# dongxianzhe/hydrainfer

Hardware: AMD Instinct MI355X
Metric: decode output tokens/s, LLaVA-1.5-7B image+text requests (576 image + 128 text prompt, 256 generated), batch 32 per GPU (higher is better)
Workload: dtype bf16; 1 GPU; LLaVA-1.5-7B-shaped random weights, batch 32 decode, paged KV block_size=16, 613 steps in 3 passes of consecutive contexts (the generation's 705..959, the last pass ctx 781..883), the state rewound between passes outside the clock (BASELINE configs[1]: LLaVA-1.5-7B bf16, collocated prefill+decode on 1 MI355X); global_batch=32, hip_graph=False, step_executor=plan, parallelism=replicas x1 (independent requests, no data-path collective)

## Files before the change

### hydrainfer_amd/csrc/gemm_xreg.hip

```cpp
#include <algorithm>
#include <cstdio>
#include <cstdlib>
#include <cstring>
#include <type_traits>
#include "attn_common.h"

namespace {

using namespace hx;

struct XregParams {
  const void* x;
  const void* w;
  float* partial;
  int64_t ldx;
  int32_t M, N, K;
  int32_t stagger;
  int32_t x_packed;
  const float* nm_partial;
  void* nm_residual;
  const void* nm_weight;
  uint32_t* sync;
  int32_t nm_splits;
  float nm_eps;
  void* act;
  int32_t interleaved;
  int32_t pk_P;
};

struct XregHot {
  const void *p0, *p1, *p2, *p3, *p4;
  int32_t a, b, c, ldx;
};
template <int NORM>
inline bool xreg_hot(const XregParams& p, unsigned nb, XregHot* h) {
  if ((p.N >> 4) > 0xffff || nb > 0xffff || (p.K >> 5) > 0xffff || p.M > 255 || p.nm_splits > 255 || p.stagger > 255 ||
      p.pk_P > 0xffff || p.pk_P < 0 || p.ldx > 0x7fffffff || p.ldx < 0)
    return false;
  h->p0 = p.w;
  if (NORM) { h->p1 = p.nm_partial; h->p2 = p.nm_residual; h->p3 = p.nm_weight; h->p4 = p.sync; }
  else { h->p1 = p.x; h->p2 = p.partial; h->p3 = p.act; h->p4 = nullptr; }
  h->a = (int32_t)((uint32_t)(p.N >> 4) | (nb << 16));
  h->b = (int32_t)((uint32_t)(p.K >> 5) | ((uint32_t)p.M << 16) | ((uint32_t)(p.x_packed ? 1 : 0) << 24) | ((uint32_t)(p.interleaved ? 1 : 0) << 25));
  h->c = (int32_t)((uint32_t)p.stagger | ((uint32_t)p.nm_splits << 8) | ((uint32_t)p.pk_P << 16));
  h->ldx = NORM ? __builtin_bit_cast(int32_t, p.nm_eps) : (int32_t)p.ldx;
  return true;
}

#define HX_XREG_HOT_SIG                                                                                             \
  const void* __restrict__ h_p0, const void* __restrict__ h_p1, const void* __restrict__ h_p2,                        \
      const void* __restrict__ h_p3, const void* __restrict__ h_p4, const int32_t h_a, const int32_t h_b,            \
      const int32_t h_c, const int32_t h_ldx
#define HX_XREG_UNPACK_HOT(NORM_)                                                                                   \
  XregParams p = p_in;                                                                                              \
  p.w = h_p0;                                                                                                       \
  if (NORM_) {                                                                                                      \
    p.nm_partial = reinterpret_cast<const float*>(h_p1); p.nm_residual = const_cast<void*>(h_p2); p.nm_weight = h_p3; \
    p.sync = reinterpret_cast<uint32_t*>(const_cast<void*>(h_p4));                                                  \
  } else {                                                                                                          \
    p.x = h_p1; p.partial = reinterpret_cast<float*>(const_cast<void*>(h_p2)); p.act = const_cast<void*>(h_p3);     \
  }                                                                                                                 \
  p.N = (h_a & 0xffff) << 4; p.K = (h_b & 0xffff) << 5; p.M = (h_b >> 16) & 0xff; p.x_packed = (h_b >> 24) & 1;     \
  p.interleaved = (h_b >> 25) & 1; p.stagger = h_c & 0xff; p.nm_splits = (h_c >> 8) & 0xff;                         \
  p.pk_P = (int32_t)((uint32_t)h_c >> 16);                                                                          \
  if (NORM_) p.nm_eps = __builtin_bit_cast(float, h_ldx);                                                           \
  else p.ldx = h_ldx;                                                                                               \
  const int h_nb = (int)((uint32_t)h_a >> 16);

__device__ __forceinline__ float silu_f32(float x) { return x / (1.0f + __expf(-x)); }

__device__ __attribute__((aligned(128))) u16 g_zero_line[64] = {0};

static_assert(HX_XREG_SYNC_WORDS >= 320 + 32, "sync area: word 0 arrivals, word 1 error, word 32*(1+xcc) the flag line of that XCD");
constexpr int kXAux = 16;
constexpr int kStateWord = 320;
constexpr uint64_t kRescueTicks = 3000;
constexpr int kMaxG = 16;

typedef __amdgpu_buffer_rsrc_t rsrc_t;
typedef unsigned int bu32x4 __attribute__((__vector_size__(16)));
__device__ __forceinline__ rsrc_t make_rsrc(const void* p) {
  return __builtin_amdgcn_make_buffer_rsrc(const_cast<void*>(p), 0, 0x7fffffff, 0x00020000);
}

template <typename T, int MAXV, int MB, int KB = 6>
__device__ __forceinline__ bool norm_row_256(const float* __restrict__ partial, int n_splits, int64_t slab_stride,
                                             u16* __restrict__ residual, const u16* __restrict__ weight, float eps,
                                             int hidden, int row, void* x_frag, uint32_t* state, float* red,
                                             int mb_layout = MB) {
  const int tid = threadIdx.x;
  const int nvec = hidden / 8;
  uint32_t claimed = 1;
  if (tid == 0) claimed = __hip_atomic_exchange(state + row, 1u, __ATOMIC_RELAXED, __HIP_MEMORY_SCOPE_AGENT);
  u16x8* res_v = reinterpret_cast<u16x8*>(residual + (int64_t)row * hidden);
  const u16x8* w_v = reinterpret_cast<const u16x8*>(weight);
  float x[2 * MAXV][8];
  float ss[2] = {0.f, 0.f};
  u16x8 rr[2 * MAXV], ww[2 * MAXV], hh[2 * MAXV];
#pragma unroll
  for (int v = 0; v < 2; ++v)
#pragma unroll
    for (int j = 0; j < MAXV; ++j) {
      const int i = min(tid + 256 * v + 512 * j, nvec - 1);
      rr[v * MAXV + j] = res_v[i];
      ww[v * MAXV + j] = w_v[i];
    }
#pragma unroll
  for (int v = 0; v < 2; ++v) {
#pragma unroll
    for (int j = 0; j < MAXV; ++j) {
      const int i = tid + 256 * v + 512 * j;
      if (i < nvec) {
        const float* pp = partial + (int64_t)row * hidden + i * 8;
        constexpr int kB = KB;
        f32x4 a = {0.f, 0.f, 0.f, 0.f}, b = {0.f, 0.f, 0.f, 0.f};
        for (int s0 = 0; s0 < n_splits; s0 += kB) {
          f32x4 pa[kB], pb[kB];
#pragma unroll
          for (int k = 0; k < kB; ++k) {
            const int sp = min(s0 + k, n_splits - 1);
            pa[k] = *reinterpret_cast<const f32x4*>(pp + sp * slab_stride);
            pb[k] = *reinterpret_cast<const f32x4*>(pp + sp * slab_stride + 4);
          }
#pragma unroll
          for (int k = 0; k < kB; ++k) {
            if (s0 + k == 0) { a = pa[0]; b = pb[0]; }
            else if (s0 + k < n_splits) { a += pa[k]; b += pb[k]; }
          }
        }
        const u16x8 r = rr[v * MAXV + j];
        u16x8 h;
#pragma unroll
        for (int e = 0; e < 8; ++e) {
          const float sum = round_to<T>(round_to<T>(e < 4 ? a[e] : b[e - 4]) + T::to_float(r[e]));
          x[v * MAXV + j][e] = sum;
          h[e] = T::from_float(sum);
          ss[v] += sum * sum;
        }
        hh[v * MAXV + j] = h;
      }
    }
  }
  const float t0 = wave_sum(ss[0]), t1 = wave_sum(ss[1]);
  if ((tid & 63) == 0) {
    red[tid >> 6] = t0;
    red[4 + (tid >> 6)] = t1;
  }
  if (tid == 0) red[8] = claimed == 0u ? 1.f : 0.f;
  __syncthreads();
  const bool own = red[8] != 0.f;
  float total = 0.f;
#pragma unroll
  for (int k = 0; k < 8; ++k) total += red[k];
  const float inv = rsqrtf(total / (float)hidden + eps);
  if (own) {
    const rsrc_t xrs = make_rsrc(x_frag);
#pragma unroll
    for (int v = 0; v < 2; ++v) {
#pragma unroll
      for (int j = 0; j < MAXV; ++j) {
        const int i = tid + 256 * v + 512 * j;
        if (i < nvec) {
          res_v[i] = hh[v * MAXV + j];
          const u16x8 w = ww[v * MAXV + j];
          u16x8 o;
#pragma unroll
          for (int e = 0; e < 8; ++e)
            o[e] = T::from_float(round_to<T>(x[v * MAXV + j][e] * inv) * T::to_float(w[e]));
          const uint32_t piece = (uint32_t)((i >> 2) * mb_layout + (row >> 4)) * 64 + (i & 3) * 16 + (row & 15);
          __builtin_amdgcn_raw_buffer_store_b128(__builtin_bit_cast(bu32x4, o), xrs, piece * 16, 0, 16);
        }
      }
    }
  }
  __syncthreads();
  return own;
}

template <typename T, int MB, int KW, int EPI = 0, int DBG = 0, int NORM = 0, int RM = 0>
__global__ __launch_bounds__(256) void gemm_xreg_kernel(HX_XREG_HOT_SIG, const XregParams p_in) {
  HX_XREG_UNPACK_HOT(NORM)
  extern __shared__ __attribute__((aligned(16))) char smem[];
  constexpr int NBUF = (KW + 7) / 8;
  constexpr int P = 4 * KW;
  const int lane = threadIdx.x & 63;
  const int w = __builtin_amdgcn_readfirstlane(threadIdx.x >> 6);
  const int g = lane >> 4, c = lane & 15;
  const int split = blockIdx.y, nb = h_nb, b = nb - 1 - (int)blockIdx.x;
  const int total_ks = p.K >> 5;
  const int n_rg = p.N >> 4;
  const int ks0 = split * P;
  const int nks = min(P, total_ks - ks0);
  const int kw = max(0, min(KW, nks - w * KW));
  const int G = EPI ? 2 * (((n_rg >> 1) - b + nb - 1) / nb) : (n_rg - b + nb - 1) / nb;
  auto rg_of = [&](int i) { return EPI ? 2 * (b + (i >> 1) * nb) + (i & 1) : b + i * nb; };
  const int j0 = (p.stagger & 1) ? (int)(((unsigned)b * 7u + (unsigned)w * 3u) % (unsigned)KW) : 0;
  const int flat_id = blockIdx.y * nb + blockIdx.x;
  auto stamp = [&](int k) {
    if (NORM && (p.stagger & 8) && threadIdx.x == 0 && (flat_id == 0 || flat_id == (int)(nb * (NORM ? 1u : gridDim.y)) - 1))
      reinterpret_cast<unsigned long long*>(p.sync + 384 + (flat_id ? 32 : 0))[k] = __builtin_amdgcn_s_memrealtime();
  };
  stamp(0);

  auto rot = [&](int t) { const int r = j0 + t; return r >= KW ? r - KW : r; };
  constexpr int64_t jstride = RM ? 32 : 512;
  const u16* wbase = RM ? reinterpret_cast<const u16*>(p.w) + (int64_t)c * p.K + 8 * g + (int64_t)ks0 * 32
                        : reinterpret_cast<const u16*>(p.w) + 8 * lane + ((int64_t)ks0 * n_rg) * 512;
  auto rg_off = [&](int rg) -> int64_t {
    if constexpr (!RM) return (int64_t)rg * nks * 512;
    else if (EPI || p.interleaved) return ((int64_t)(rg & 1) * (p.N >> 1) + (int64_t)(rg >> 1) * 16) * p.K;
    else return (int64_t)rg * 16 * p.K;
  };
  const int wave_k0 = min(w * KW, max(nks - 1, 0));
  auto frag_ptr = [&](int rg, int t) {
    const int r = rot(t);
    const int j = wave_k0 + (r < kw ? r : 0);
    return wbase + rg_off(rg) + j * jstride;
  };

  u16x8 buf[NBUF][8];
  auto load_buf = [&](int rg, int q) {
#pragma unroll
    for (int j = 0; j < 8; ++j)
      if (8 * q + j < KW) buf[q][j] = __builtin_nontemporal_load(reinterpret_cast<const u16x8*>(frag_ptr(rg, 8 * q + j)));
  };
  u16x8 xb[KW][MB];
  const u16* xp = reinterpret_cast<const u16*>(p.x) + 8 * g;
  const u16* zp = reinterpret_cast<const u16*>(g_zero_line) + 8 * g;
  auto load_x_block = [&](int q) {
#pragma unroll
    for (int j = 0; j < 8; ++j) {
      const int t = 8 * q + j;
      if (t < KW) {
        const int r = rot(t);
        const bool ok = r < kw;
        const int ks = min(ks0 + w * KW + r, total_ks - 1);
#pragma unroll
        for (int mb = 0; mb < MB; ++mb) {
          const int m = min(mb * 16 + c, p.M - 1);
          const u16* src = ok ? (p.x_packed ? reinterpret_cast<const u16*>(p.x) + ((int64_t)(ks * MB + mb) * 64 + lane) * 8
                                            : xp + (int64_t)m * p.ldx + (int64_t)ks * 32)
                              : zp;
          if (DBG & 1) xb[t][mb] = u16x8{1, 2, 3, 4, 5, 6, (u16)t, (u16)lane};
          else xb[t][mb] = *reinterpret_cast<const u16x8*>(src);
        }
      }
    }
  };
  if (NORM) {
    uint32_t* st = p.sync + kStateWord;
    float* red = reinterpret_cast<float*>(smem);
    int* cmd = reinterpret_cast<int*>(smem) + 16;
    auto produce = [&](int row) {
      const bool own = norm_row_256<T, (KW + 31) / 32, MB>(p.nm_partial, p.nm_splits, (int64_t)p.M * p.K,
                                                           reinterpret_cast<u16*>(p.nm_residual),
                                                           reinterpret_cast<const u16*>(p.nm_weight), p.nm_eps, p.K, row,
                                                           const_cast<void*>(p.x), st, red);
      if (own) {
        asm volatile("s_waitcnt vmcnt(0)" ::: "memory");
        __syncthreads();
        if (threadIdx.x == 0) {
          const uint32_t old = __hip_atomic_fetch_add(p.sync, 1u, __ATOMIC_RELAXED, __HIP_MEMORY_SCOPE_AGENT);
          if (old + 1 == (uint32_t)p.M) {
#pragma unroll
            for (int cpy = 0; cpy < 8; ++cpy)
              __hip_atomic_store(p.sync + 32 * (1 + cpy), 1u, __ATOMIC_RELAXED, __HIP_MEMORY_SCOPE_AGENT);
          }
        }
      }
      return own;
    };
    const int flat = flat_id;
    const int n_wg = nb;
    if (flat < p.M && !(p.stagger & 6))
      for (int row = flat; row < p.M; row += n_wg) produce(row);
    stamp(1);
#pragma unroll
    for (int q = 0; q < NBUF; ++q) load_buf(rg_of(0), q);
    __builtin_amdgcn_sched_barrier(0);
    for (;;) {
      if (threadIdx.x < 64) {
        const uint32_t* fl = p.sync + 32 * (1 + (__builtin_amdgcn_s_getreg(20 | (3 << 11)) & 7));
        const uint64_t t0 = __builtin_amdgcn_s_memrealtime();
        int c = -1;
        while (!__builtin_amdgcn_readfirstlane(__hip_atomic_load(fl, __ATOMIC_RELAXED, __HIP_MEMORY_SCOPE_AGENT))) {
          __builtin_amdgcn_s_sleep(8);
          const uint64_t waited = __builtin_amdgcn_s_memrealtime() - t0;
          if (waited > kRescueTicks && !(p.stagger & 4)) {
            const uint32_t sv = lane < p.M ? __hip_atomic_load(st + lane, __ATOMIC_RELAXED, __HIP_MEMORY_SCOPE_AGENT) : 1u;
            uint64_t free_rows = __ballot(sv == 0u);
            if (free_rows) {
              for (int skip = flat % __builtin_popcountll(free_rows); skip > 0; --skip) free_rows &= free_rows - 1;
              c = __builtin_ctzll(free_rows);
              break;
            }
          }
          if (waited > ((p.stagger & 4) ? 200000ull : 100000000ull)) {
            if (threadIdx.x == 0) __hip_atomic_fetch_or(p.sync + 1, 1u, __ATOMIC_RELAXED, __HIP_MEMORY_SCOPE_AGENT);
            c = -2;
            break;
          }
        }
        if (threadIdx.x == 0) *cmd = c;
      }
      __syncthreads();
      const int c = *cmd;
      __syncthreads();
      if (c < 0) break;
      produce(c);
    }
    stamp(2);
    asm volatile("" ::: "memory");
    {
      const rsrc_t xrs = make_rsrc(p.x), zrs = make_rsrc(g_zero_line);
#pragma unroll
      for (int t = 0; t < KW; ++t) {
        const int r = rot(t);
        const bool ok = r < kw;
        const int ks = min(ks0 + w * KW + r, total_ks - 1);
#pragma unroll
        for (int mb = 0; mb < MB; ++mb) {
          xb[t][mb] = __builtin_bit_cast(u16x8, __builtin_amdgcn_raw_buffer_load_b128(
              ok ? xrs : zrs, ok ? (uint32_t)((ks * MB + mb) * 64 + lane) * 16 : (uint32_t)(lane & 7) * 16, 0, kXAux));
        }
      }
    }
    __builtin_amdgcn_sched_barrier(0);
  } else {
#pragma unroll
    for (int q = 0; q < NBUF; ++q) {
      load_x_block(q);
      load_buf(rg_of(0), q);
      __builtin_amdgcn_sched_barrier(0);
    }
  }

  f32x4 acc[MB];
#pragma unroll
  for (int mb = 0; mb < MB; ++mb) acc[mb] = f32x4{0.f, 0.f, 0.f, 0.f};
  f32x4* slot = reinterpret_cast<f32x4*>(smem) + (w * MB) * 64 + lane;

  auto row_group = [&](int i, auto refill_tag) {
    constexpr bool REFILL = decltype(refill_tag)::value;
    const int rg_next = rg_of(i + 1);
#pragma unroll
    for (int q = 0; q < NBUF; ++q) {
#pragma unroll
      for (int j = 0; j < 8; ++j) {
        if (8 * q + j < KW) {
#pragma unroll
          for (int mb = 0; mb < MB; ++mb) acc[mb] = Mfma<T>::mma(buf[q][j], xb[8 * q + j][mb], acc[mb]);
        }
      }
      __builtin_amdgcn_sched_barrier(0);
      if (REFILL) load_buf(rg_next, q);
      __builtin_amdgcn_sched_barrier(0);
    }
#pragma unroll
    for (int mb = 0; mb < MB; ++mb) {
      slot[(i * 4 * MB + mb) * 64] = acc[mb];
      acc[mb] = f32x4{0.f, 0.f, 0.f, 0.f};
    }
  };
  for (int i = 0; i < G - 1; ++i) { row_group(i, std::true_type{}); if (i < 6) stamp(3 + i); }
  row_group(G - 1, std::false_type{});
  stamp(10);
  if ((DBG & 2) && acc[0][0] != 123.25f) return;
  __syncthreads();

  const f32x4* tiles = reinterpret_cast<const f32x4*>(smem) + lane;
  auto tile_sum = [&](int i, int mb) {
    f32x4 s = tiles[((i * 4 + 0) * MB + mb) * 64];
#pragma unroll
    for (int ww = 1; ww < 4; ++ww) s += tiles[((i * 4 + ww) * MB + mb) * 64];
    return s;
  };
  if (EPI == 0) {
    for (int pr = w; pr < G * MB; pr += 4) {
      const int i = pr / MB, mb = pr - i * MB;
      const f32x4 s = tile_sum(i, mb);
      const int m = mb * 16 + c;
      const int rg = rg_of(i);
      const int col = p.interleaved ? ((rg & 1) ? (p.N >> 1) : 0) + ((rg >> 1) << 4) : (rg << 4);
      if (m < p.M) *reinterpret_cast<f32x4*>(p.partial + ((int64_t)split * p.M + m) * p.N + col + 4 * g) = s;
    }
  } else {
    for (int pr = w; pr < (G >> 1) * MB; pr += 4) {
      const int ip = pr / MB, mb = pr - ip * MB;
      const f32x4 gt = tile_sum(2 * ip, mb), up = tile_sum(2 * ip + 1, mb);
      u16x4 r;
#pragma unroll
      for (int e = 0; e < 4; ++e)
        r[e] = T::from_float(round_to<T>(silu_f32(round_to<T>(gt[e]))) * round_to<T>(up[e]));
      const int k = 16 * (b + ip * nb) + 4 * g;
      u16* dst = reinterpret_cast<u16*>(p.act) + ((((int64_t)(k >> 5) * MB + mb) * 64 + ((k & 31) >> 3) * 16 + c) << 3) + (k & 7);
      *reinterpret_cast<u16x4*>(dst) = r;
    }
  }
  stamp(11);
}

template <typename T, int KW, int NORM, int RG = 2, int EPI = 0>
__global__ __launch_bounds__(256) void gemm_xreg_wide_kernel(HX_XREG_HOT_SIG, const XregParams p_in) {
  HX_XREG_UNPACK_HOT(NORM)
  extern __shared__ __attribute__((aligned(16))) char smem[];
  constexpr int MB = 4, NBUF = (KW + 7) / 8, P = 4 * KW;
  static_assert(!EPI || (RG == 2 && NORM == 1), "the two-pass form: (gate, up) pairs, norm-fused");
  const int lane = threadIdx.x & 63;
  const int w = __builtin_amdgcn_readfirstlane(threadIdx.x >> 6);
  const int g = lane >> 4, c = lane & 15;
  const int split = EPI ? 0 : (int)blockIdx.y, nb = h_nb, b = nb - 1 - (int)blockIdx.x;
  const int total_ks = p.K >> 5;
  const int n_rg = p.N >> 4, n_un = n_rg / RG;
  const int sp = split >> 1, off_in = (split & 1) * P;
  const int nks_p = min(p.pk_P, total_ks - sp * p.pk_P);
  const int ks0 = sp * p.pk_P + off_in;
  const int nks = max(0, min(P, nks_p - off_in));
  const int kw = max(0, min(KW, nks - w * KW));
  const int G = (n_un - b + nb - 1) / nb;
  const int mbl = (p.M + 15) >> 4;
  const int j0 = (p.stagger & 1) ? (int)(((unsigned)b * 7u + (unsigned)w * 3u) % (unsigned)KW) : 0;
  const int flat_id = blockIdx.y * nb + blockIdx.x;
  auto stamp = [&](int k) {
    if (NORM && (p.stagger & 8) && threadIdx.x == 0 && (flat_id == 0 || flat_id == (int)(nb * gridDim.y) - 1))
      reinterpret_cast<unsigned long long*>(p.sync + 384 + (flat_id ? 32 : 0))[k] = __builtin_amdgcn_s_memrealtime();
  };
  stamp(0);
  auto rot = [&](int t) { const int r = j0 + t; return r >= KW ? r - KW : r; };
  const u16* wbase = reinterpret_cast<const u16*>(p.w) + 8 * lane + ((int64_t)sp * p.pk_P * n_rg) * 512;
  const int wave_k0 = off_in + min(w * KW, max(nks - 1, 0));
  struct PassK { int ks0, kw, wk0; };
  const PassK pa{ks0, kw, wave_k0};
  const int nks_b = max(0, min(P, nks_p - P));
  const PassK pb{ks0 + P, max(0, min(KW, nks_b - w * KW)), P + min(w * KW, max(nks_b - 1, 0))};
  auto frag_ptr = [&](int rg, int t, const PassK& ps) {
    const int r = rot(t);
    return wbase + ((int64_t)rg * nks_p + ps.wk0 + (r < ps.kw ? r : 0)) * 512;
  };
  u16x8 buf[RG][NBUF][8];
  auto load_buf = [&](int unit, int q, const PassK& ps) {
#pragma unroll
    for (int h = 0; h < RG; ++h)
#pragma unroll
      for (int j = 0; j < 8; ++j)
        if (8 * q + j < KW)
          buf[h][q][j] = __builtin_nontemporal_load(reinterpret_cast<const u16x8*>(frag_ptr(RG * unit + h, 8 * q + j, ps)));
  };
  auto unit_of = [&](int i) { return b + i * nb; };
  u16x8 xb[KW][MB];
  const u16* xp = reinterpret_cast<const u16*>(p.x) + 8 * g;
  const u16* zp = reinterpret_cast<const u16*>(g_zero_line) + 8 * g;
  auto load_x_block = [&](int q) {
#pragma unroll
    for (int j = 0; j < 8; ++j) {
      const int t = 8 * q + j;
      if (t < KW) {
        const int r = rot(t);
        const bool ok = r < kw;
        const int ks = min(ks0 + w * KW + r, total_ks - 1);
#pragma unroll
        for (int mb = 0; mb < MB; ++mb) {
          const int m = min(mb * 16 + c, p.M - 1);
          const u16* src = ok ? (p.x_packed ? reinterpret_cast<const u16*>(p.x) + ((int64_t)(ks * mbl + min(mb, mbl - 1)) * 64 + lane) * 8
                                            : xp + (int64_t)m * p.ldx + (int64_t)ks * 32)
                              : zp;
          xb[t][mb] = *reinterpret_cast<const u16x8*>(src);
        }
      }
    }
  };
  if (NORM) {
    uint32_t* st = p.sync + kStateWord;
    float* red = reinterpret_cast<float*>(smem);
    int* cmd = reinterpret_cast<int*>(smem) + 16;
    auto produce = [&](int row) {
      const bool own = norm_row_256<T, (2 * KW + 31) / 32, MB, 8>(p.nm_partial, p.nm_splits, (int64_t)p.M * p.K,
                                                               reinterpret_cast<u16*>(p.nm_residual),
                                                               reinterpret_cast<const u16*>(p.nm_weight), p.nm_eps, p.K, row,
                                                               const_cast<void*>(p.x), st, red, mbl);
      if (own) {
        asm volatile("s_waitcnt vmcnt(0)" ::: "memory");
        __syncthreads();
        if (threadIdx.x == 0) {
          const uint32_t old = __hip_atomic_fetch_add(p.sync, 1u, __ATOMIC_RELAXED, __HIP_MEMORY_SCOPE_AGENT);
          if (old + 1 == (uint32_t)p.M) {
#pragma unroll
            for (int cpy = 0; cpy < 8; ++cpy)
              __hip_atomic_store(p.sync + 32 * (1 + cpy), 1u, __ATOMIC_RELAXED, __HIP_MEMORY_SCOPE_AGENT);
          }
        }
      }
      return own;
    };
    const int n_wg = nb * (int)gridDim.y;
    if (flat_id < p.M && !(p.stagger & 6))
      for (int row = flat_id; row < p.M; row += n_wg) produce(row);
#pragma unroll
    for (int q = 0; q < NBUF; ++q) load_buf(unit_of(0), q, pa);
    __builtin_amdgcn_sched_barrier(0);
    stamp(1);
    for (;;) {
      if (threadIdx.x < 64) {
        const uint32_t* fl = p.sync + 32 * (1 + (__builtin_amdgcn_s_getreg(20 | (3 << 11)) & 7));
        const uint64_t t0 = __builtin_amdgcn_s_memrealtime();
        int cc = -1;
        while (!__builtin_amdgcn_readfirstlane(__hip_atomic_load(fl, __ATOMIC_RELAXED, __HIP_MEMORY_SCOPE_AGENT))) {
          __builtin_amdgcn_s_sleep(8);
          const uint64_t waited = __builtin_amdgcn_s_memrealtime() - t0;
          if (waited > kRescueTicks && !(p.stagger & 4)) {
            const uint32_t sv = lane < p.M ? __hip_atomic_load(st + lane, __ATOMIC_RELAXED, __HIP_MEMORY_SCOPE_AGENT) : 1u;
            uint64_t free_rows = __ballot(sv == 0u);
            if (free_rows) {
              for (int skip = flat_id % __builtin_popcountll(free_rows); skip > 0; --skip) free_rows &= free_rows - 1;
              cc = __builtin_ctzll(free_rows);
              break;
            }
          }
          if (waited > ((p.stagger & 4) ? 200000ull : 100000000ull)) {
            if (threadIdx.x == 0) __hip_atomic_fetch_or(p.sync + 1, 1u, __ATOMIC_RELAXED, __HIP_MEMORY_SCOPE_AGENT);
            cc = -2;
            break;
          }
        }
        if (threadIdx.x == 0) *cmd = cc;
      }
      __syncthreads();
      const int cc = *cmd;
      __syncthreads();
      if (cc < 0) break;
      produce(cc);
    }
    stamp(2);
    asm volatile("" ::: "memory");
  }
  auto load_x_norm = [&](const PassK& ps) {
    const rsrc_t xrs = make_rsrc(p.x), zrs = make_rsrc(g_zero_line);
#pragma unroll
    for (int t = 0; t < KW; ++t) {
      const int r = rot(t);
      const bool ok = r < ps.kw;
      const int ks = min(ps.ks0 + w * KW + r, total_ks - 1);
#pragma unroll
      for (int mb = 0; mb < MB; ++mb)
        xb[t][mb] = __builtin_bit_cast(u16x8, __builtin_amdgcn_raw_buffer_load_b128(
            ok ? xrs : zrs, ok ? (uint32_t)((ks * mbl + min(mb, mbl - 1)) * 64 + lane) * 16 : (uint32_t)(lane & 7) * 16, 0, kXAux));
    }
  };
  if (NORM) {
    load_x_norm(pa);
    __builtin_amdgcn_sched_barrier(0);
  } else {
#pragma unroll
    for (int q = 0; q < NBUF; ++q) {
      load_x_block(q);
      load_buf(unit_of(0), q, pa);
      __builtin_amdgcn_sched_barrier(0);
    }
  }

  f32x4 acc[RG][MB];
#pragma unroll
  for (int h = 0; h < RG; ++h)
#pragma unroll
    for (int mb = 0; mb < MB; ++mb) acc[h][mb] = f32x4{0.f, 0.f, 0.f, 0.f};
  f32x4* tiles = reinterpret_cast<f32x4*>(smem) + lane;
  auto mfma_unit = [&](auto refill_tag, int u_next, const PassK& ps_next) {
    constexpr bool REFILL = decltype(refill_tag)::value;
#pragma unroll
    for (int q = 0; q < NBUF; ++q) {
#pragma unroll
      for (int j = 0; j < 8; ++j) {
        if (8 * q + j < KW) {
#pragma unroll
          for (int h = 0; h < RG; ++h)
#pragma unroll
            for (int mb = 0; mb < MB; ++mb) acc[h][mb] = Mfma<T>::mma(buf[h][q][j], xb[8 * q + j][mb], acc[h][mb]);
        }
      }
      __builtin_amdgcn_sched_barrier(0);
      if (REFILL) load_buf(u_next, q, ps_next);
      __builtin_amdgcn_sched_barrier(0);
    }
  };
  auto reduce_unit = [&](int set, f32x4 (&sum)[RG]) {
#pragma unroll
    for (int h = 0; h < RG; ++h)
#pragma unroll
      for (int mb = 0; mb < MB; ++mb) {
        tiles[(((set * RG + h) * 4 + w) * MB + mb) * 64] = acc[h][mb];
        acc[h][mb] = f32x4{0.f, 0.f, 0.f, 0.f};
      }
    __syncthreads();
#pragma unroll
    for (int k = 0; k < RG; ++k) {
      const int tt = w + 4 * k, h = tt >> 2, mb = tt & 3;
      sum[k] = tiles[(((set * RG + h) * 4 + 0) * MB + mb) * 64];
#pragma unroll
      for (int ww = 1; ww < 4; ++ww) sum[k] += tiles[(((set * RG + h) * 4 + ww) * MB + mb) * 64];
    }
  };
  if constexpr (!EPI) {
    auto unit = [&](int i, auto refill_tag) {
      mfma_unit(refill_tag, unit_of(i + 1), pa);
      f32x4 sum[RG];
      reduce_unit(i & 1, sum);
#pragma unroll
      for (int k = 0; k < RG; ++k) {
        const int tt = w + 4 * k, h = tt >> 2, mb = tt & 3;
        const int rg = RG * unit_of(i) + h;
        const int col = p.interleaved ? ((rg & 1) ? (p.N >> 1) : 0) + ((rg >> 1) << 4) : (rg << 4);
        const int m = mb * 16 + c;
        if (m < p.M) *reinterpret_cast<f32x4*>(p.partial + ((int64_t)split * p.M + m) * p.N + col + 4 * g) = sum[k];
      }
    };
    for (int i = 0; i < G - 1; ++i) { unit(i, std::true_type{}); if (i < 6) stamp(3 + i); }
    unit(G - 1, std::false_type{});
  } else {
    f32x4* part = reinterpret_cast<f32x4*>(smem + 2 * RG * 4 * MB * 1024) + lane;
    int n_red = 0;
    for (int i = 0; i < G; ++i) {
      const bool seam = i + 1 == G;
      mfma_unit(std::true_type{}, seam ? unit_of(0) : unit_of(i + 1), seam ? pb : pa);
      f32x4 sum[RG];
      reduce_unit(n_red++ & 1, sum);
#pragma unroll
      for (int k = 0; k < RG; ++k) part[((i * RG + k) * 4 + w) * 64] = sum[k];
      if (i < 3) stamp(3 + i);
    }
    load_x_norm(pb);
    __builtin_amdgcn_sched_barrier(0);
    auto finish = [&](int i, auto refill_tag) {
      mfma_unit(refill_tag, unit_of(i + 1), pb);
      f32x4 sum[RG];
      reduce_unit(n_red++ & 1, sum);
      f32x4 gt = part[((i * RG + 0) * 4 + w) * 64], up = part[((i * RG + 1) * 4 + w) * 64];
      gt += sum[0];
      up += sum[1];
      const int m = w * 16 + c;
      if (m < p.M) {
        u16x4 r;
#pragma unroll
        for (int e = 0; e < 4; ++e)
          r[e] = T::from_float(round_to<T>(silu_f32(round_to<T>(gt[e]))) * round_to<T>(up[e]));
        const int k = (unit_of(i) << 4) + 4 * g;
        u16* dst = reinterpret_cast<u16*>(p.act) + ((((int64_t)(k >> 5) * mbl + w) * 64 + ((k & 31) >> 3) * 16 + c) << 3) + (k & 7);
        *reinterpret_cast<u16x4*>(dst) = r;
      }
    };
    for (int i = 0; i < G - 1; ++i) { finish(i, std::true_type{}); if (i < 3) stamp(6 + i); }
    finish(G - 1, std::false_type{});
  }
  stamp(11);
}

__global__ __launch_bounds__(256) void pack_xreg_kernel(u16* __restrict__ packed, const u16* __restrict__ w,
                                                        int64_t n_pieces, int total_ks, int n_rg, int64_t ldw, int P,
                                                        int interleave) {
  const int64_t i = (int64_t)blockIdx.x * 256 + threadIdx.x;
  if (i >= n_pieces) return;
  const int lane = (int)(i & 63);
  const int64_t blk = i >> 6;
  const int64_t per_split = (int64_t)P * n_rg;
  const int split = (int)(blk / per_split);
  const int ks0 = split * P;
  const int nks = min(P, total_ks - ks0);
  const int64_t rem = blk - (int64_t)ks0 * n_rg;
  const int64_t rg = rem / nks;
  const int s = ks0 + (int)(rem % nks);
  const int64_t srg = interleave ? (rg >> 1) + ((rg & 1) ? (n_rg >> 1) : 0) : rg;
  const u16* src = w + (16 * srg + (lane & 15)) * ldw + 32 * s + 8 * (lane >> 4);
  *reinterpret_cast<u16x8*>(packed + i * 8) = *reinterpret_cast<const u16x8*>(src);
}

int g_stagger = 1;
int g_no_producers = 0;
int g_dbg = 0;
int g_row_major = 0;
int g_timeline = 0;
int g_force_wgs = 0;

constexpr int kKwSet[] = {4, 8, 16, 20, 22, 27, 29, 32, 40};

int round_kw(int kw) {
  for (int v : kKwSet) if (v >= kw) return v;
  return 0;
}

int n_cus() {
  static int n = [] {
    int dev = 0;
    hipDeviceProp_t prop;
    if (hipGetDevice(&dev) != hipSuccess || hipGetDeviceProperties(&prop, dev) != hipSuccess) return 256;
    return prop.multiProcessorCount > 0 ? prop.multiProcessorCount : 256;
  }();
  return n;
}

void xreg_plan(int64_t N, int64_t K, int* S, int* KW, bool fewest_splits = false) {
  const int total_ks = (int)(K >> 5);
  const int n_rg = (int)(N >> 4);
  const int s0 = (total_ks + 159) / 160;
  auto kw_of = [&](int s) { return round_kw(((total_ks + s - 1) / s + 3) / 4); };
  auto wgs_of = [&](int s) {
    int nb = n_cus() / s;
    if (nb < 1) nb = 1;
    if (nb > n_rg) nb = n_rg;
    const int G = (n_rg + nb - 1) / nb;
    return s * ((n_rg + G - 1) / G);
  };
  int s = s0;
  if (!fewest_splits) {
    auto waste_pct = [&](int sc) {
      const int kw = kw_of(sc);
      if (kw <= 0) return 1000;
      const int used = (total_ks + 4 * kw - 1) / (4 * kw);
      return used != sc ? 1000 : (int)(((int64_t)used * 4 * kw * 100) / total_ks) - 100;
    };
    const int w0 = waste_pct(s0), w1 = waste_pct(s0 + 1);
    if (w1 <= 4 && (w0 > 4 ||
                    (wgs_of(s0) * 5 < n_cus() * 4 && wgs_of(s0 + 1) > wgs_of(s0))))
      s = s0 + 1;
  }
  static const char* env = getenv("HX_XREG_S");
  if (env) {
    const char* q = env;
    while (*q) {
      long k = 0, sv = 0;
      if (sscanf(q, "%ld:%ld", &k, &sv) == 2 && k == K && sv >= s0 && sv <= 16) s = (int)sv;
      const char* semi = strchr(q, ';');
      if (!semi) break;
      q = semi + 1;
    }
  }
  *KW = kw_of(s);
  *S = *KW > 0 ? (total_ks + 4 * *KW - 1) / (4 * *KW) : 0;
}

template <typename T, int MB, int KW, int EPI, int NORM = 0>
int launch_kw(const XregParams& p, int S, hipStream_t stream) {
  const int n_units = EPI ? (p.N >> 5) : (p.N >> 4);
  const int per_unit = EPI ? 2 : 1;
  const int cap = g_force_wgs > 0 ? g_force_wgs : n_cus();
  int nb = cap / S;
  if (nb < 1) nb = 1;
  if (nb > n_units) nb = n_units;
  int G = (n_units + nb - 1) / nb;
  if (G * per_unit > kMaxG) {
    G = kMaxG / per_unit;
    nb = (n_units + G - 1) / G;
  }
  if (((n_units + nb - 1) / nb) * per_unit > kMaxG) return HX_ERR_SHAPE;
  const size_t lds = (size_t)G * per_unit * 4 * MB * 1024;
  if (lds > 48 * 1024) {
    hipError_t e = hipFuncSetAttribute((const void*)gemm_xreg_kernel<T, MB, KW, EPI, 0, NORM>,
                                       hipFuncAttributeMaxDynamicSharedMemorySize, (int)lds);
    if (e != hipSuccess) return hip_rc(e);
  }
  const dim3 grid((unsigned)nb, (unsigned)S);
  XregHot h;
  if (!xreg_hot<NORM>(p, (unsigned)nb, &h)) return HX_ERR_SHAPE;
  if (NORM && S != 1) return HX_ERR_SHAPE;
#define HX_XREG_LAUNCH(...) hx::launcher(gemm_xreg_kernel<__VA_ARGS__>, grid, 256, lds, stream)(h.p0, h.p1, h.p2, h.p3, h.p4, h.a, h.b, h.c, h.ldx, p)
  if constexpr (EPI == 0 && NORM == 0 && MB == 2 && (KW == 32 || KW == 29)) if (g_dbg) {
    if (g_dbg == 1) HX_XREG_LAUNCH(T, MB, KW, 0, 1);
    else if (g_dbg == 2) HX_XREG_LAUNCH(T, MB, KW, 0, 2);
    else HX_XREG_LAUNCH(T, MB, KW, 0, 3);
    return check_launch();
  }
#if HX_EXPERIMENTS
  if constexpr (MB == 2 && (KW == 32 || KW == 22 || KW == 29)) if (p.stagger & 16) {
    HX_XREG_LAUNCH(T, MB, KW, EPI, 0, NORM, 1);
    return check_launch();
  }
#endif
  HX_XREG_LAUNCH(T, MB, KW, EPI, 0, NORM);
#undef HX_XREG_LAUNCH
  return check_launch();
}

template <typename T, int MB, int EPI, int NORM = 0>
int launch_mb(const XregParams& p, int S, int KW, hipStream_t stream) {
  switch (KW) {
    case 4: return launch_kw<T, MB, 4, EPI, NORM>(p, S, stream);
    case 8: return launch_kw<T, MB, 8, EPI, NORM>(p, S, stream);
    case 16: return launch_kw<T, MB, 16, EPI, NORM>(p, S, stream);
    case 20: if constexpr (EPI == 0 && NORM == 0) return launch_kw<T, MB, 20, 0>(p, S, stream); else return HX_ERR_SHAPE;
    case 22: if constexpr (EPI == 0 && NORM == 0) return launch_kw<T, MB, 22, 0>(p, S, stream); else return HX_ERR_SHAPE;
    case 27: if constexpr (EPI == 0 && NORM == 0) return launch_kw<T, MB, 27, 0>(p, S, stream); else return HX_ERR_SHAPE;
    case 29: if constexpr (EPI == 0 && NORM == 0) return launch_kw<T, MB, 29, 0>(p, S, stream); else return HX_ERR_SHAPE;
    case 32: return launch_kw<T, MB, 32, EPI, NORM>(p, S, stream);
    case 40: return launch_kw<T, MB, 40, EPI, NORM>(p, S, stream);
    default: return HX_ERR_SHAPE;
  }
}

template <int EPI, int NORM = 0>
int launch_any(const XregParams& p, int S, int KW, int dtype, hipStream_t stream) {
  const int MB = (p.M + 15) / 16;
  if (dtype == HX_F16) return MB == 1 ? launch_mb<F16, 1, EPI, NORM>(p, S, KW, stream) : launch_mb<F16, 2, EPI, NORM>(p, S, KW, stream);
  return MB == 1 ? launch_mb<BF16, 1, EPI, NORM>(p, S, KW, stream) : launch_mb<BF16, 2, EPI, NORM>(p, S, KW, stream);
}

bool wide_plan(int64_t N, int64_t K, bool gate_up_packing, int* S, int* KW, int* pkP, int* S_packed) {
  if (N <= 0 || K <= 0 || N % 32 || K % 32) return false;
  int sp, kwp;
  xreg_plan(N, K, &sp, &kwp, gate_up_packing);
  if (kwp <= 0) return false;
  const int kw = (kwp + 1) / 2;
  if (kw != 2 && kw != 4 && kw != 8 && kw != 10 && kw != 11 && kw != 14 && kw != 16 && kw != 20) return false;
  const int total_ks = (int)(K >> 5);
  int n = 0;
  for (int q = 0; q < sp; ++q) {
    const int nks_p = std::min(4 * kwp, total_ks - q * 4 * kwp);
    n += nks_p > 4 * kw ? 2 : 1;
  }
  *KW = kw; *pkP = 4 * kwp; *S = n; *S_packed = sp;
  return true;
}

constexpr int wide_rg(int kw) { return kw == 20 ? 1 : 2; }

template <typename T, int KW, int NORM, int EPI = 0>
int launch_wide_kw(const XregParams& p, int S, hipStream_t stream) {
  constexpr int RG = wide_rg(KW);
  const int n_units = (int)(p.N >> 4) / RG;
  if (EPI) S = 1;
  int nb = n_cus() / S;
  if (nb < 1) nb = 1;
  if (nb > n_units) nb = n_units;
  size_t lds = 2 * RG * 4 * 4 * 1024;
  if (EPI) lds += (size_t)((n_units + nb - 1) / nb) * RG * 4 * 1024;
  if (lds > 150 * 1024) return HX_ERR_SHAPE;
  {
    hipError_t e = hipFuncSetAttribute((const void*)gemm_xreg_wide_kernel<T, KW, NORM, RG, EPI>,
// ... 359 lines not shown
```

Baseline: 6557 tokens/s.

## Replace block-wide flag wait with per-wave scalar polling and shared handover

The fused norm+GEMM kernel used to wait for the norm-ready flag with wave 0 polling and then two block barriers. Each wave now polls the flag itself with scalar glc loads. A small shared-memory handshake word escalates to a block barrier only when wave 0 decides to rescue a free row or give up. This is meant to remove the barrier round-trip from the common path so waves can start their GEMM as soon as the flag rises. In exchange it brings more complex cross-wave coordination with possible race risk, and more scalar memory traffic from every wave polling.

```diff
diff --git a/hydrainfer_amd/csrc/gemm_xreg.hip b/hydrainfer_amd/csrc/gemm_xreg.hip
--- a/hydrainfer_amd/csrc/gemm_xreg.hip
+++ b/hydrainfer_amd/csrc/gemm_xreg.hip
@@ -175,6 +175,75 @@
   }
   __syncthreads();
   return own;
+}
+
+__device__ __forceinline__ uint32_t flag_poll_scalar(const uint32_t* fl) {
+  uint32_t v;
+  asm volatile("s_load_dword %0, %1, 0x0 glc\n\ts_waitcnt lgkmcnt(0)" : "=&s"(v) : "s"(fl) : "memory");
+  return v;
+}
+constexpr int kCmdGaveUp = 1, kCmdFlagUp = 2, kCmdRow0 = 3;
+template <typename Produce>
+__device__ __forceinline__ void handover_wait(const XregParams& p, int w, int lane, int flat, uint32_t* st, int* hs,
+                                              Produce&& produce) {
+  const uint32_t* fl = p.sync + 32 * (1 + (__builtin_amdgcn_s_getreg(20 | (3 << 11)) & 7));
+  for (;;) {
+    bool slow = false;
+    if (w == 0) {
+      const uint64_t t0 = __builtin_amdgcn_s_memrealtime();
+      while (!flag_poll_scalar(fl)) {
+        __builtin_amdgcn_s_sleep(8);
+        const uint64_t waited = __builtin_amdgcn_s_memrealtime() - t0;
+        int d = 0;
+        if (waited > kRescueTicks) {
+          if (__builtin_amdgcn_readfirstlane(__hip_atomic_load(fl, __ATOMIC_RELAXED, __HIP_MEMORY_SCOPE_AGENT))) {
+            d = kCmdFlagUp;
+          } else if (!(p.stagger & 4)) {
+            const uint32_t sv = lane < p.M ? __hip_atomic_load(st + lane, __ATOMIC_RELAXED, __HIP_MEMORY_SCOPE_AGENT) : 1u;
+            uint64_t free_rows = __ballot(sv == 0u);
+            if (free_rows) {
+              for (int skip = flat % __builtin_popcountll(free_rows); skip > 0; --skip) free_rows &= free_rows - 1;
+              d = kCmdRow0 + __builtin_ctzll(free_rows);
+            }
+          }
+        }
+        if (!d && waited > ((p.stagger & 4) ? 200000ull : 100000000ull)) d = kCmdGaveUp;
+        if (d) {
+          int seen = 0;
+          if (lane == 0) {
+            __hip_atomic_compare_exchange_strong(hs, &seen, 2, __ATOMIC_RELAXED, __ATOMIC_RELAXED, __HIP_MEMORY_SCOPE_WORKGROUP);
+            if (seen == 0) {
+              if (d == kCmdGaveUp) __hip_atomic_fetch_or(p.sync + 1, 1u, __ATOMIC_RELAXED, __HIP_MEMORY_SCOPE_AGENT);
+              __hip_atomic_store(hs + 1, d, __ATOMIC_RELAXED, __HIP_MEMORY_SCOPE_WORKGROUP);
+            }
+          }
+          slow = __builtin_amdgcn_readfirstlane(seen) == 0;
+          break;
+        }
+      }
+    } else {
+      for (;;) {
+        if (flag_poll_scalar(fl)) {
+          int old = 0;
+          if (lane == 0) old = __hip_atomic_fetch_or(hs, 1, __ATOMIC_RELAXED, __HIP_MEMORY_SCOPE_WORKGROUP);
+          slow = (__builtin_amdgcn_readfirstlane(old) & 2) != 0;
+          break;
+        }
+        if (__builtin_amdgcn_readfirstlane(__hip_atomic_load(hs + 1, __ATOMIC_RELAXED, __HIP_MEMORY_SCOPE_WORKGROUP))) {
+          slow = true;
+          break;
+        }
+        __builtin_amdgcn_s_sleep(8);
+      }
+    }
+    if (!slow) return;
+    __syncthreads();
+    const int cmd = hs[1];
+    __syncthreads();
+    if (threadIdx.x == 0) { hs[0] = 0; hs[1] = 0; }
+    if (cmd < kCmdRow0) return;
+    produce(cmd - kCmdRow0);
+  }
 }
 
 template <typename T, int MB, int KW, int EPI = 0, int DBG = 0, int NORM = 0, int RM = 0>
@@ -250,7 +319,8 @@
   if (NORM) {
     uint32_t* st = p.sync + kStateWord;
     float* red = reinterpret_cast<float*>(smem);
-    int* cmd = reinterpret_cast<int*>(smem) + 16;
+    __shared__ int hs[2];
+    if (threadIdx.x == 0) { hs[0] = 0; hs[1] = 0; }
     auto produce = [&](int row) {
       const bool own = norm_row_256<T, (KW + 31) / 32, MB>(p.nm_partial, p.nm_splits, (int64_t)p.M * p.K,
                                                            reinterpret_cast<u16*>(p.nm_residual),
@@ -268,6 +338,7 @@
           }
         }
       }
+      __builtin_amdgcn_s_waitcnt(0x0f70);
       return own;
     };
     const int flat = flat_id;
@@ -278,37 +349,8 @@
 #pragma unroll
     for (int q = 0; q < NBUF; ++q) load_buf(rg_of(0), q);
     __builtin_amdgcn_sched_barrier(0);
-    for (;;) {
-      if (threadIdx.x < 64) {
-        const uint32_t* fl = p.sync + 32 * (1 + (__builtin_amdgcn_s_getreg(20 | (3 << 11)) & 7));
-        const uint64_t t0 = __builtin_amdgcn_s_memrealtime();
-        int c = -1;
-        while (!__builtin_amdgcn_readfirstlane(__hip_atomic_load(fl, __ATOMIC_RELAXED, __HIP_MEMORY_SCOPE_AGENT))) {
-          __builtin_amdgcn_s_sleep(8);
-          const uint64_t waited = __builtin_amdgcn_s_memrealtime() - t0;
-          if (waited > kRescueTicks && !(p.stagger & 4)) {
-            const uint32_t sv = lane < p.M ? __hip_atomic_load(st + lane, __ATOMIC_RELAXED, __HIP_MEMORY_SCOPE_AGENT) : 1u;
-            uint64_t free_rows = __ballot(sv == 0u);
-            if (free_rows) {
-              for (int skip = flat % __builtin_popcountll(free_rows); skip > 0; --skip) free_rows &= free_rows - 1;
-              c = __builtin_ctzll(free_rows);
-              break;
-            }
-          }
-          if (waited > ((p.stagger & 4) ? 200000ull : 100000000ull)) {
-            if (threadIdx.x == 0) __hip_atomic_fetch_or(p.sync + 1, 1u, __ATOMIC_RELAXED, __HIP_MEMORY_SCOPE_AGENT);
-            c = -2;
-            break;
-          }
-        }
-        if (threadIdx.x == 0) *cmd = c;
-      }
-      __syncthreads();
-      const int c = *cmd;
-      __syncthreads();
-      if (c < 0) break;
-      produce(c);
-    }
+    __syncthreads();
+    handover_wait(p, w, lane, flat, st, hs, produce);
     stamp(2);
     asm volatile("" ::: "memory");
     {
@@ -472,7 +514,8 @@
   if (NORM) {
     uint32_t* st = p.sync + kStateWord;
     float* red = reinterpret_cast<float*>(smem);
-    int* cmd = reinterpret_cast<int*>(smem) + 16;
+    __shared__ int hs[2];
+    if (threadIdx.x == 0) { hs[0] = 0; hs[1] = 0; }
     auto produce = [&](int row) {
       const bool own = norm_row_256<T, (2 * KW + 31) / 32, MB, 8>(p.nm_partial, p.nm_splits, (int64_t)p.M * p.K,
                                                                reinterpret_cast<u16*>(p.nm_residual),
@@ -490,6 +533,7 @@
           }
         }
       }
+      __builtin_amdgcn_s_waitcnt(0x0f70);
       return own;
     };
     const int n_wg = nb * (int)gridDim.y;
@@ -498,38 +542,9 @@
 #pragma unroll
     for (int q = 0; q < NBUF; ++q) load_buf(unit_of(0), q, pa);
     __builtin_amdgcn_sched_barrier(0);
+    __syncthreads();
     stamp(1);
-    for (;;) {
-      if (threadIdx.x < 64) {
-        const uint32_t* fl = p.sync + 32 * (1 + (__builtin_amdgcn_s_getreg(20 | (3 << 11)) & 7));
-        const uint64_t t0 = __builtin_amdgcn_s_memrealtime();
-        int cc = -1;
-        while (!__builtin_amdgcn_readfirstlane(__hip_atomic_load(fl, __ATOMIC_RELAXED, __HIP_MEMORY_SCOPE_AGENT))) {
-          __builtin_amdgcn_s_sleep(8);
-          const uint64_t waited = __builtin_amdgcn_s_memrealtime() - t0;
-          if (waited > kRescueTicks && !(p.stagger & 4)) {
-            const uint32_t sv = lane < p.M ? __hip_atomic_load(st + lane, __ATOMIC_RELAXED, __HIP_MEMORY_SCOPE_AGENT) : 1u;
-            uint64_t free_rows = __ballot(sv == 0u);
-            if (free_rows) {
-              for (int skip = flat_id % __builtin_popcountll(free_rows); skip > 0; --skip) free_rows &= free_rows - 1;
-              cc = __builtin_ctzll(free_rows);
-              break;
-            }
-          }
-          if (waited > ((p.stagger & 4) ? 200000ull : 100000000ull)) {
-            if (threadIdx.x == 0) __hip_atomic_fetch_or(p.sync + 1, 1u, __ATOMIC_RELAXED, __HIP_MEMORY_SCOPE_AGENT);
-            cc = -2;
-            break;
-          }
-        }
-        if (threadIdx.x == 0) *cmd = cc;
-      }
-      __syncthreads();
-      const int cc = *cmd;
-      __syncthreads();
-      if (cc < 0) break;
-      produce(cc);
-    }
+    handover_wait(p, w, lane, flat_id, st, hs, produce);
     stamp(2);
     asm volatile("" ::: "memory");
   }
```

Result: slower. 6061 tokens/s (-7.6%).
